# cloudflare/circl

Hardware: AMD Instinct MI355X
Metric: ML-KEM-768 encapsulations/sec (whole node), batch=2^20 (higher is better)
Workload: dtype i32; 1 GPU; ML-KEM-768 Encapsulate, distinct-key (one GPU-generated key per item), batch=1048576 per GPU, inputs resident in HBM (SURVEY 8d scope i; the PCIe-inclusive host-ABI rate, scope ii, is `value_host_abi`); key_pool=1048576, parallelism=batch split per device, no collectives, mode=encaps

## Files before the change

circl_amd/csrc/api_prims.hip:

```cpp
#include "host_common.h"
#include "prim_kernels.h"
#include "sampler_prims.h"

using namespace circl::host;

namespace {
PipeOpts prim_opts(size_t row_bytes) {
    PipeOpts o;
    o.chunk_items = host_chunk_items(std::max<size_t>(size_t(1) << 10, (size_t(32) << 20) / std::max<size_t>(row_bytes, 1)));
    return o;
}
const std::function<size_t(size_t)> no_ws = [](size_t) { return size_t(0); };
}

extern "C" {

int circl_hip_keccak_f1600(uint64_t *states, size_t n, int rounds, int device) {
    if (rounds != 24 && rounds != 12) return CIRCL_HIP_EPARAM;
    uint8_t *p = reinterpret_cast<uint8_t *>(states);
    return shard(n, device, [&](int dev, size_t lo, size_t cnt) {
        return run_pipeline(dev, cnt, {{p + lo * 200, 200}}, {}, {{p + lo * 200, 200}}, no_ws, prim_opts(200), [&](Chunk &c) {
            HIP_TRY(hipMemcpyAsync(c.out[0], c.in[0], c.cnt * 200, hipMemcpyDeviceToDevice, c.st));
            hipLaunchKernelGGL(circl::prim::keccak_f1600_kernel, dim3((unsigned)((c.cnt + 255) / 256)), dim3(256), 0, c.st,
                               reinterpret_cast<uint64_t *>(c.out[0]), c.cnt, 24 - rounds);
// ... 21 lines not shown
    auto timed = [&](auto kern, int iters, double insts_per_wave, double *out) -> int {
        float best = 1e30f;
        for (int rep = 0; rep < 4; rep++) {
            HIP_TRY(hipEventRecord(a, st));
            hipLaunchKernelGGL(kern, dim3((unsigned)(cus * waves_per_simd)), dim3(256), 0, st, sink, iters);
            HIP_TRY(hipEventRecord(b, st));
            HIP_TRY(hipEventSynchronize(b));
            float ms = 0;
            HIP_TRY(hipEventElapsedTime(&ms, a, b));
            if (rep > 0) best = std::min(best, ms);
        }
        if (out) *out = insts_per_wave * waves_per_simd / (best * 1e-3);
        return CIRCL_HIP_OK;
    };
    int rc = CIRCL_HIP_OK;
    if (hipEventCreate(&a) != hipSuccess || hipEventCreate(&b) != hipSuccess || hipStreamCreateWithFlags(&st, hipStreamNonBlocking) != hipSuccess) {
        (void)hipGetLastError();
        rc = CIRCL_HIP_EHIP;
    }
    constexpr int kKeccakIters = 512, kSimpleIters = 8192;
    if (rc == CIRCL_HIP_OK) rc = timed(circl::prim::keccak_rate_probe_kernel, kKeccakIters, 4320.0 * kKeccakIters, keccak_insts_per_s_per_simd);
    if (rc == CIRCL_HIP_OK) rc = timed(circl::prim::simple_rate_probe_kernel, kSimpleIters, (double)circl::prim::kSimpleProbePerIter * kSimpleIters, simple_insts_per_s_per_simd);
    cleanup();
    return rc;
}

int circl_hip_keccak_f1600_coop(uint64_t *states, size_t n, int device) {
    uint8_t *p = reinterpret_cast<uint8_t *>(states);
    return shard(n, device, [&](int dev, size_t lo, size_t cnt) {
        return run_pipeline(dev, cnt, {{p + lo * 200, 200}}, {}, {{p + lo * 200, 200}}, no_ws, prim_opts(200), [&](Chunk &c) {
            HIP_TRY(hipMemcpyAsync(c.out[0], c.in[0], c.cnt * 200, hipMemcpyDeviceToDevice, c.st));
            hipLaunchKernelGGL(circl::prim::keccak_f1600_coop_kernel, dim3((unsigned)c.cnt), dim3(64), 0, c.st, reinterpret_cast<uint64_t *>(c.out[0]));
            HIP_TRY(hipGetLastError());
            return CIRCL_HIP_OK;
        });
    });
}

int circl_hip_keccak_f1600_split(uint64_t *states, size_t n, int device) {
    uint8_t *p = reinterpret_cast<uint8_t *>(states);
    return shard(n, device, [&](int dev, size_t lo, size_t cnt) {
        return run_pipeline(dev, cnt, {{p + lo * 200, 200}}, {}, {{p + lo * 200, 200}}, no_ws, prim_opts(200), [&](Chunk &c) {
            HIP_TRY(hipMemcpyAsync(c.out[0], c.in[0], c.cnt * 200, hipMemcpyDeviceToDevice, c.st));
            hipLaunchKernelGGL(circl::prim::keccak_f1600_split_kernel, dim3((unsigned)((2 * c.cnt + 255) / 256)), dim3(256), 0, c.st,
                               reinterpret_cast<uint64_t *>(c.out[0]), c.cnt);
            HIP_TRY(hipGetLastError());
            return CIRCL_HIP_OK;
        });
    });
}

int circl_hip_kyber_ntt(int16_t *polys, size_t n, int inverse, int device) {
    uint8_t *p = reinterpret_cast<uint8_t *>(polys);
    return shard(n, device, [&](int dev, size_t lo, size_t cnt) {
        return run_pipeline(dev, cnt, {{p + lo * 512, 512}}, {}, {{p + lo * 512, 512}}, no_ws, prim_opts(512), [&](Chunk &c) {
            HIP_TRY(hipMemcpyAsync(c.out[0], c.in[0], c.cnt * 512, hipMemcpyDeviceToDevice, c.st));
            hipLaunchKernelGGL(circl::prim::kyber_ntt_kernel, dim3((unsigned)c.cnt), dim3(64), 0, c.st, reinterpret_cast<int16_t *>(c.out[0]), inverse);
            HIP_TRY(hipGetLastError());
            return CIRCL_HIP_OK;
        });
    });
}

int circl_hip_dilithium_ntt(uint32_t *polys, size_t n, int inverse, int device) {
    uint8_t *p = reinterpret_cast<uint8_t *>(polys);
    return shard(n, device, [&](int dev, size_t lo, size_t cnt) {
        return run_pipeline(dev, cnt, {{p + lo * 1024, 1024}}, {}, {{p + lo * 1024, 1024}}, no_ws, prim_opts(1024), [&](Chunk &c) {
            HIP_TRY(hipMemcpyAsync(c.out[0], c.in[0], c.cnt * 1024, hipMemcpyDeviceToDevice, c.st));
            hipLaunchKernelGGL(circl::prim::dilithium_ntt_kernel, dim3((unsigned)c.cnt), dim3(64), 0, c.st, reinterpret_cast<uint32_t *>(c.out[0]), inverse);
            HIP_TRY(hipGetLastError());
            return CIRCL_HIP_OK;
        });
    });
}

int circl_hip_kyber_mulhat(int16_t *out, const int16_t *a, const int16_t *b, size_t n, int device) {
    uint8_t *po = reinterpret_cast<uint8_t *>(out);
    const uint8_t *pa = reinterpret_cast<const uint8_t *>(a), *pb = reinterpret_cast<const uint8_t *>(b);
    return shard(n, device, [&](int dev, size_t lo, size_t cnt) {
        return run_pipeline(dev, cnt, {{pa + lo * 512, 512}, {pb + lo * 512, 512}}, {}, {{po + lo * 512, 512}}, no_ws, prim_opts(512), [&](Chunk &c) {
            hipLaunchKernelGGL(circl::prim::kyber_mulhat_kernel, dim3((unsigned)c.cnt), dim3(64), 0, c.st, reinterpret_cast<int16_t *>(c.out[0]),
                               reinterpret_cast<const int16_t *>(c.in[0]), reinterpret_cast<const int16_t *>(c.in[1]));
            HIP_TRY(hipGetLastError());
            return CIRCL_HIP_OK;
        });
    });
}

int circl_hip_shake(int rate, int ds, const uint8_t *in, size_t inlen, uint8_t *out, size_t outlen, size_t n, int device) {
    if ((rate != 168 && rate != 136 && rate != 72) || (ds != 0x1f && ds != 0x06) || outlen == 0) return CIRCL_HIP_EPARAM;
    const size_t il = inlen ? inlen : 1;
    std::vector<uint8_t> pad;
    const uint8_t *src = in;
    if (!inlen) { pad.assign(n, 0); src = pad.data(); }
    return shard(n, device, [&](int dev, size_t lo, size_t cnt) {
        return run_pipeline(dev, cnt, {{src + lo * il, il}}, {}, {{out + lo * outlen, outlen}}, no_ws, prim_opts(il + outlen), [&](Chunk &c) {
            hipLaunchKernelGGL(circl::prim::sponge_kernel, dim3((unsigned)((c.cnt + 255) / 256)), dim3(256), 0, c.st, rate / 8, (uint32_t)ds, 0,
                               (const uint8_t *)c.in[0], inlen, (const uint64_t *)nullptr, c.out[0], outlen, c.cnt);
            HIP_TRY(hipGetLastError());
            return CIRCL_HIP_OK;
        });
    });
}

int circl_hip_lane_op(int op, int arg, const uint32_t *a, const uint32_t *b, uint32_t *out0, uint32_t *out1, size_t n, int device) {
    if (op < 1 || op >= CIRCL_HIP_LANE_OP_COUNT || !a || !out0) return CIRCL_HIP_EPARAM;
    const uint8_t *pa = reinterpret_cast<const uint8_t *>(a), *pb = reinterpret_cast<const uint8_t *>(b);
    uint8_t *p0 = reinterpret_cast<uint8_t *>(out0), *p1 = reinterpret_cast<uint8_t *>(out1);
    return shard(n, device, [&](int dev, size_t lo, size_t cnt) {
        std::vector<HIn> ins = {{pa + lo * 4, 4}};
// ... 233 lines not shown
```

circl_amd/csrc/kyber_dev.h:

```cpp
#pragma once
#include "keccak_dev.h"

namespace circl {
namespace kyber {

constexpr int Q = 3329;
constexpr int N = 256;

CIRCL_HD int mul24(int a, int b) {
#if defined(__HIP_DEVICE_COMPILE__)
    return __mul24(a, b);
#else
    return a * b;
#endif
}
CIRCL_HD uint32_t umulhi32(uint32_t a, uint32_t b) {
#if defined(__HIP_DEVICE_COMPILE__)
    return __umulhi(a, b);
#else
    return (uint32_t)(((uint64_t)a * b) >> 32);
#endif
}

CIRCL_HD int barrett(int x) { return x - mul24(mul24(x, 20159) >> 26, Q); }
CIRCL_HD int csubq(int x) {
    x -= Q;
    return x + ((x >> 31) & Q);
}
CIRCL_HD int normalize(int x) { return csubq(barrett(x)); }

constexpr uint32_t qinv32() {
    uint32_t x = 1;
    for (int i = 0; i < 6; i++) x = x * (2u - (uint32_t)Q * x);
    return x;
}
constexpr uint32_t QINV32 = qinv32();
static_assert((uint32_t)(QINV32 * (uint32_t)Q) == 1u, "q * qinv == 1 mod 2^32");
constexpr uint32_t R32 = (uint32_t)((1ull << 32) % Q);
constexpr uint32_t MULC_LIMIT = (uint32_t)((1ull << 32) / Q);
constexpr uint32_t modq(int64_t x) { return (uint32_t)(((x % Q) + Q) % Q); }
constexpr uint32_t powq(uint32_t b, uint32_t e) {
    uint32_t r = 1;
    for (uint32_t i = 0; i < e; i++) r = r * b % Q;
    return r;
}
constexpr uint32_t invq(uint32_t x) { return powq(x % Q, Q - 2); }
constexpr uint32_t mulc_const(uint32_t w) { return modq(-(int64_t)((uint64_t)(w % Q) * R32 % Q)) * QINV32; }
CIRCL_HD uint32_t mulc(uint32_t b, uint32_t c) { return umulhi32(b * c, (uint32_t)Q); }
CIRCL_HD uint32_t reduce32(uint32_t t) { return umulhi32(t * QINV32, (uint32_t)Q); }
constexpr uint32_t NEG_R32 = modq(-(int64_t)R32);

struct ZetaTable {
    uint32_t w[128];
    uint32_t c[128];
// ... 21 lines not shown
CIRCL_HD uint32_t zeta_plain(int i) {
    constexpr ZetaTable t = make_zetas();
    return t.w[i];
}

struct LaneZetas {
    uint32_t f2, f3a, f3b, f4, f5a, f5b, f6, f6n;
    uint32_t i2, i3a, i3b, i4, i5a, i5b, i6;
};
CIRCL_HD LaneZetas load_lane_zetas(int lane) {
    LaneZetas z;
    const int h = lane >> 4, m = lane >> 2;
    z.f2 = zeta_c(4 + h);
    z.f3a = zeta_c(8 + 2 * h);
    z.f3b = zeta_c(9 + 2 * h);
    z.f4 = zeta_c(16 + m);
    z.f5a = zeta_c(32 + 2 * m);
    z.f5b = zeta_c(33 + 2 * m);
    z.f6 = zeta_c(64 + lane);
    z.f6n = zeta_cn(64 + lane);
    z.i2 = zeta_c(7 - h);
    z.i3a = zeta_c(15 - 2 * h);
    z.i3b = zeta_c(14 - 2 * h);
    z.i4 = zeta_c(31 - m);
    z.i5a = zeta_c(63 - 2 * m);
    z.i5b = zeta_c(62 - 2 * m);
    z.i6 = zeta_c(127 - lane);
    return z;
}

CIRCL_HD int idx_l1(int l, int r) { return l + 64 * r; }
CIRCL_HD int idx_l2(int l, int r) { return ((l >> 4) << 6) | (r << 4) | (l & 15); }
CIRCL_HD int idx_l3(int l, int r) { return ((l >> 2) << 4) | (r << 2) | (l & 3); }
CIRCL_HD int idx_l4(int l, int r) { return 4 * l + r; }

CIRCL_HD void ct(int &a, int &b, uint32_t c) {
    const int t = (int)mulc((uint32_t)b, c);
    b = a + Q - t;
    a = a + t;
}
template <int BOUND> CIRCL_HD void gs(int &a, int &b, uint32_t c) {
    const int t = b + BOUND - a;
    a = a + b;
    b = (int)mulc((uint32_t)t, c);
}

#if defined(__HIP_DEVICE_COMPILE__) || defined(__HIPCC__)

template <bool NW = false> __device__ __forceinline__ void wave_sync() {
    if constexpr (NW) wave_lds_order();
    else __syncthreads();
}

template <int FROM, int TO, class T, bool NW = false> __device__ __forceinline__ void relayout(int (&c)[4], void *xch_raw, int lane) {
    T *xch = reinterpret_cast<T *>(xch_raw);
    auto idx = [&](int which, int r) {
        return which == 1 ? idx_l1(lane, r) : which == 2 ? idx_l2(lane, r) : which == 3 ? idx_l3(lane, r) : idx_l4(lane, r);
    };
    wave_sync<NW>();
#pragma unroll
    for (int r = 0; r < 4; r++) xch[idx(FROM, r)] = (T)c[r];
    wave_sync<NW>();
#pragma unroll
    for (int r = 0; r < 4; r++) c[r] = (int)xch[idx(TO, r)];
}

template <bool NW = false> __device__ __forceinline__ void ntt(int (&c)[4], const LaneZetas &z, void *xch, int lane) {
    const uint32_t z1 = zeta_c(1), z2 = zeta_c(2), z3 = zeta_c(3);
    ct(c[0], c[2], z1); ct(c[1], c[3], z1);
    ct(c[0], c[1], z2); ct(c[2], c[3], z3);
    relayout<1, 2, uint16_t, NW>(c, xch, lane);
    ct(c[0], c[2], z.f2); ct(c[1], c[3], z.f2);
    ct(c[0], c[1], z.f3a); ct(c[2], c[3], z.f3b);
    relayout<2, 3, uint16_t, NW>(c, xch, lane);
    ct(c[0], c[2], z.f4); ct(c[1], c[3], z.f4);
    ct(c[0], c[1], z.f5a); ct(c[2], c[3], z.f5b);
    relayout<3, 4, uint16_t, NW>(c, xch, lane);
    ct(c[0], c[2], z.f6); ct(c[1], c[3], z.f6);
}

template <uint32_t SCALE, bool NW = false> __device__ __forceinline__ void invntt(int (&c)[4], const LaneZetas &z, void *xch, int lane) {
    static_assert(128u * Q < MULC_LIMIT, "lazy sums stay inside the mulc domain");
    gs<Q>(c[0], c[2], z.i6); gs<Q>(c[1], c[3], z.i6);
    relayout<4, 3, uint16_t, NW>(c, xch, lane);
    gs<2 * Q>(c[0], c[1], z.i5a); gs<2 * Q>(c[2], c[3], z.i5b);
    gs<4 * Q>(c[0], c[2], z.i4); gs<4 * Q>(c[1], c[3], z.i4);
    relayout<3, 2, uint16_t, NW>(c, xch, lane);
    gs<8 * Q>(c[0], c[1], z.i3a); gs<8 * Q>(c[2], c[3], z.i3b);
    gs<16 * Q>(c[0], c[2], z.i2); gs<16 * Q>(c[1], c[3], z.i2);
    relayout<2, 1, uint32_t, NW>(c, xch, lane);
    const uint32_t z1 = zeta_c(1), z2 = zeta_c(2), z3 = zeta_c(3);
    gs<32 * Q>(c[0], c[1], z3); gs<32 * Q>(c[2], c[3], z2);
    gs<64 * Q>(c[0], c[2], z1); gs<64 * Q>(c[1], c[3], z1);
    constexpr uint32_t fin = mulc_const((uint32_t)((uint64_t)(SCALE % Q) * invq(128) % Q));
#pragma unroll
    for (int r = 0; r < 4; r++) c[r] = (int)mulc((uint32_t)c[r], fin);
}
#endif

struct HatOperand {
    uint32_t p0, q0, p1, q1;
};
CIRCL_HD uint32_t pack16(int lo, int hi) { return ((uint32_t)lo & 0xffffu) | ((uint32_t)hi << 16); }
CIRCL_HD HatOperand hat_prepare(const int (&b)[4], uint32_t c_zeta, uint32_t c_neg_zeta) {
    HatOperand h;
    h.p0 = pack16(b[0], (int)mulc((uint32_t)b[1], c_zeta));
    h.q0 = pack16(b[1], b[0]);
    h.p1 = pack16(b[2], (int)mulc((uint32_t)b[3], c_neg_zeta));
    h.q1 = pack16(b[3], b[2]);
    return h;
}
CIRCL_HD int dot2(uint32_t a, uint32_t b, int c) {
#if defined(__HIP_DEVICE_COMPILE__)
    typedef short short2v __attribute__((ext_vector_type(2)));
    return __builtin_amdgcn_sdot2(__builtin_bit_cast(short2v, a), __builtin_bit_cast(short2v, b), c, false);
#else
    return (int)(int16_t)(a & 0xffff) * (int)(int16_t)(b & 0xffff) + (int)(int16_t)(a >> 16) * (int)(int16_t)(b >> 16) + c;
#endif
}
CIRCL_HD void mulhat_acc_packed(int (&acc)[4], uint32_t a01, uint32_t a23, const HatOperand &b) {
    acc[0] = dot2(a01, b.p0, acc[0]);
    acc[1] = dot2(a01, b.q0, acc[1]);
    acc[2] = dot2(a23, b.p1, acc[2]);
    acc[3] = dot2(a23, b.q1, acc[3]);
}
CIRCL_HD void mulhat_finish(int (&acc)[4]) {
#pragma unroll
    for (int r = 0; r < 4; r++) acc[r] = (int)reduce32((uint32_t)acc[r]);
}

CIRCL_HD int cbd2_from_nibble(unsigned t) {
    return (int)((t & 1) + ((t >> 1) & 1)) - (int)(((t >> 2) & 1) + ((t >> 3) & 1));
}
CIRCL_HD uint32_t cbd2_bias8_word(uint32_t w) {
    const uint32_t d = (w & 0x55555555u) + ((w >> 1) & 0x55555555u);
    return ((d & 0x33333333u) | 0x88888888u) - ((d >> 2) & 0x33333333u);
}
CIRCL_HD int cbd3_from_6bits(unsigned t) {
    return (int)((t & 1) + ((t >> 1) & 1) + ((t >> 2) & 1)) - (int)(((t >> 3) & 1) + ((t >> 4) & 1) + ((t >> 5) & 1));
}

template <int D> CIRCL_HD unsigned compress_coeff(int x) {
    static_assert(D == 4 || D == 5 || D == 10 || D == 11, "d");
// ... 16 lines not shown
```

circl_amd/csrc/mlkem_kernels.h:

```cpp
#pragma once
#include "kyber_dev.h"

#ifndef CIRCL_KEM_RING_PRIO
#define CIRCL_KEM_RING_PRIO 1
#endif
#ifndef CIRCL_KEM_WAVES_PER_EU
#define CIRCL_KEM_WAVES_PER_EU 4
#endif

namespace circl {
namespace mlkem {

using kyber::Q;

template <int K> struct Params;
template <> struct Params<2> { static constexpr int ETA1 = 3, DU = 10, DV = 4; };
template <> struct Params<3> { static constexpr int ETA1 = 2, DU = 10, DV = 4; };
template <> struct Params<4> { static constexpr int ETA1 = 2, DU = 11, DV = 5; };

template <int K> struct Geom {
    using P = Params<K>;
    static constexpr int EK = 384 * K + 32;
    static constexpr int DK = 768 * K + 96;
    static constexpr int CT = 32 * (P::DU * K + P::DV);
// ... 264 lines not shown
    const uint8_t *dkp = dk + idx * Gm::DK;
    KeccakState g;
    keccak_zero(g);
    xor_words<0, 4>(g, reinterpret_cast<const uint64_t *>(mprime_ws + idx * 32));
    xor_words<4, 4>(g, reinterpret_cast<const uint64_t *>(dkp + 768 * K + 32));
    g.lo[8] = kDsSha3;
    g.hi[8] = 0x80000000u;
    keccak_f1600(g);
    store_words<0, 4>(reinterpret_cast<uint64_t *>(kbar_ws + idx * 32), g);
    store_words<4, 4>(reinterpret_cast<uint64_t *>(r_ws + idx * 32), g);
    const uint64_t *zw = reinterpret_cast<const uint64_t *>(dkp + 768 * K + 64);
#pragma unroll
    for (int i = 0; i < 4; i++) reinterpret_cast<uint64_t *>(z_ws + idx * 32)[i] = zw[i];
    status[idx] = 0;
}


__device__ __forceinline__ void parse_shake128_block(const KeccakState &s, int16_t *poly, int &cnt) {
    detail::static_for<0, 112>([&](auto ic) {
        constexpr int c = decltype(ic)::v;
        constexpr int bit = 12 * c, w = bit / 32, sh = bit % 32;
        auto word = [&](int i) -> uint32_t { return (i & 1) ? s.hi[i >> 1] : s.lo[i >> 1]; };
        uint32_t v;
        if constexpr (sh <= 20) v = (word(w) >> sh) & 0xfffu;
        else v = alignbit(word(w + 1), word(w), sh) & 0xfffu;
        poly[cnt] = (int16_t)v;
        cnt = min(cnt + (v < (uint32_t)Q ? 1 : 0), 256);
    });
}

template <int K, bool TRANSPOSED>
__device__ __forceinline__ void sample_matrix(uint8_t *lds_a, const uint8_t *__restrict__ rho, size_t rho_stride, size_t item0,
                                              size_t n, int lane) {
    using Gm = Geom<K>;
    const bool on = lane < Gm::A_STREAMS;
    const int g = on ? lane / Gm::PAIRS : 0, p = on ? lane % Gm::PAIRS : 0;
    const int i = p / K, j = p % K;
    size_t item = item0 + g;
    if (item >= n) item = n - 1;
    KeccakState s;
    keccak_zero(s);
    xor_words<0, 4>(s, reinterpret_cast<const uint64_t *>(rho + item * rho_stride));
    s.lo[4] = (TRANSPOSED ? (uint32_t)i | ((uint32_t)j << 8) : (uint32_t)j | ((uint32_t)i << 8)) | (kDsShake << 16);
    s.hi[20] = 0x80000000u;
    int16_t *poly = reinterpret_cast<int16_t *>(lds_a + (on ? lane : 0) * Gm::A_STRIDE);
    int cnt = on ? 0 : 256;
#pragma unroll 1
    for (int blk = 0; blk < 3 || __any(cnt < 256); blk++) {
        keccak_f1600(s);
        if (on) parse_shake128_block(s, poly, cnt);
    }
}

template <bool TAIL, int SLOTS = 32>
__device__ __forceinline__ void parse_shake128_block_fifo(const KeccakState &s, int16_t *fifo, int16_t *row, int &cnt, int &flushed) {
    bool live = true;
    detail::static_for<0, 112>([&](auto ic) {
        constexpr int c = decltype(ic)::v;
        constexpr int bit = 12 * c, w = bit / 32, sh = bit % 32;
        auto word = [&](int i) -> uint32_t { return (i & 1) ? s.hi[i >> 1] : s.lo[i >> 1]; };
        if (!TAIL || live) {
            uint32_t v;
            if constexpr (sh <= 20) v = (word(w) >> sh) & 0xfffu;
            else v = alignbit(word(w + 1), word(w), sh) & 0xfffu;
            fifo[cnt & (SLOTS - 1)] = (int16_t)v;
            cnt += v < (uint32_t)Q ? 1 : 0;
            if constexpr (c % 8 == 7) {
                cnt = min(cnt, 256);
                if (cnt - flushed >= 8) {
                    const uint4 d = *reinterpret_cast<const uint4 *>(fifo + (flushed & (SLOTS - 1)));
                    *reinterpret_cast<uint4 *>(row + flushed) = d;
                    flushed += 8;
                }
                if constexpr (TAIL) live = __any(flushed < 256);
            }
        }
    });
}

template <int K, bool TRANSPOSED, int GA = Geom<K>::G, bool XY_ARG = false>
__device__ __forceinline__ void sample_matrix_scratch(uint8_t *lds_fifo, int16_t *rows, const uint8_t *__restrict__ rho,
                                                      size_t rho_stride, size_t item0, size_t n, int lane, const uint8_t *__restrict__ xy = nullptr) {
    using Gm = Geom<K>;
    const bool on = XY_ARG ? item0 + lane < n : lane < GA * Gm::PAIRS;
    const int g = XY_ARG ? lane : on ? lane / Gm::PAIRS : 0, p = on ? lane % Gm::PAIRS : 0;
    const int i = p / K, j = p % K;
    size_t item = item0 + g;
    if (item >= n) item = n - 1;
    KeccakState s;
    keccak_zero(s);
    xor_words<0, 4>(s, reinterpret_cast<const uint64_t *>(rho + item * rho_stride));
    if constexpr (XY_ARG) s.lo[4] = (uint32_t)xy[2 * item] | ((uint32_t)xy[2 * item + 1] << 8) | (kDsShake << 16);
    else s.lo[4] = (TRANSPOSED ? (uint32_t)i | ((uint32_t)j << 8) : (uint32_t)j | ((uint32_t)i << 8)) | (kDsShake << 16);
    s.hi[20] = 0x80000000u;
    int16_t *fifo = reinterpret_cast<int16_t *>(lds_fifo + lane * Gm::FIFO_STRIDE);
    int16_t *row = rows + lane * 256;
    int cnt = on ? 0 : 256, flushed = cnt;
#pragma unroll 1
    for (int blk = 0; blk < 3; blk++) {
        keccak_f1600(s);
        if (on) parse_shake128_block_fifo<false>(s, fifo, row, cnt, flushed);
    }
#pragma unroll 1
    while (__any(flushed < 256)) {
        keccak_f1600(s);
        parse_shake128_block_fifo<true>(s, fifo, row, cnt, flushed);
    }
}

template <bool ETA2> __device__ __forceinline__ void store_prf_words(uint32_t *out, const KeccakState &s) {
    detail::static_for<0, 16>([&](auto ic) {
        constexpr int w = decltype(ic)::v;
        out[2 * w] = ETA2 ? kyber::cbd2_bias8_word(s.lo[w]) : s.lo[w];
        out[2 * w + 1] = ETA2 ? kyber::cbd2_bias8_word(s.hi[w]) : s.hi[w];
    });
}

template <int K, bool TRANSPOSED, int NOISE, int ETA1_COUNT>
__device__ __forceinline__ void sample_matrix_and_prf(uint8_t *lds_fifo, uint8_t *lds_noise, uint8_t *lds_mini, int16_t *rows,
// ... 418 lines not shown
                __syncthreads();
                sample_matrix_scratch<K, true>(lds_a, rows, ek + 384 * K, ek_stride, item0, n, lane);
                __threadfence_block();
            } else {
                sample_matrix<K, true>(lds_a, ek + 384 * K, ek_stride, item0, n, lane);
            }
        }
        __syncthreads();
        if constexpr (Gm::HALVES == 1) {
            if (!(ABLATE & 2)) prf_streams<K, Gm::NOISE, K>(lds_noise, r_ws, 32, item0, n, lane);
            __syncthreads();
        }
    }

    int lane_ring = lane;
    asm volatile("" : "+v"(lane_ring));
    if constexpr (CIRCL_KEM_RING_PRIO != 0) __builtin_amdgcn_s_setprio(CIRCL_KEM_RING_PRIO);
    lap(1);
    const kyber::LaneZetas z = kyber::load_lane_zetas(lane_ring);
#pragma unroll 1
    for (int g = 0; g < ((ABLATE & 4) ? 0 : (int)gi); g++) {
        const size_t item = item0 + g;
        if (item >= n) break;
        if constexpr (Gm::HALVES > 1 && !SHARED) {
            if (g % Gm::GH == 0) {
                __syncthreads();
                if (!(ABLATE & 2)) prf_streams<K, Gm::NOISE, K, Gm::GH>(lds_noise, r_ws, 32, item0, n, lane, g);
                __syncthreads();
            }
        }
        const size_t kq = KM == KM_KEYED ? (key_idx ? (size_t)key_idx[item] : (ek_stride ? item : size_t(0))) : item;
        const uint8_t *ekp = ek + kq * ek_stride;
        const int16_t *krows = KM == KM_KEYED ? key_rows + kq * (size_t)(K * K * 256) : nullptr;
        const uint8_t *noise = lds_noise + (SHARED ? g : g % Gm::GH) * Gm::NOISE * Gm::NOISE_STRIDE;

        int th[K][4];
        bool bad = false;
#pragma unroll
        for (int j = 0; j < K; j++) {
            unpack12_l4(th[j], ekp + 384 * j, lane);
#pragma unroll
            for (int r = 0; r < 4; r++) {
                if (MODE == ENCAPS) bad |= th[j][r] >= Q;
                else th[j][r] = kyber::csubq(th[j][r]);
            }
        }
        const bool reject = MODE == ENCAPS ? __any(bad) : false;

        int rh[K][4];
#pragma unroll
        for (int j = 0; j < K; j++) {
#pragma unroll
            for (int r = 0; r < 4; r++) rh[j][r] = cbd_coeff<P::ETA1>(noise + j * Gm::NOISE_STRIDE, kyber::idx_l1(lane, r));
            kyber::ntt(rh[j], z, xch, lane);
        }
        kyber::HatOperand rop[K];
#pragma unroll
        for (int j = 0; j < K; j++) rop[j] = kyber::hat_prepare(rh[j], z.f6, z.f6n);

        uint8_t *ctp = ct + item * Gm::CT;
        bool differs = false;
#pragma unroll 1
        for (int i = 0; i < K; i++) {
            uint32_t *dst = reinterpret_cast<uint32_t *>(ctp + 32 * P::DU * i);
            RefWords<P::DU> ref;
            if (MODE == REENCRYPT) ref.load(dst, lane);
            int acc[4] = {0, 0, 0, 0};
#pragma unroll
            for (int j = 0; j < K; j++) {
                uint32_t a01, a23;
                if constexpr (KM == KM_KEYED) AFromCache{krows}.load(a01, a23, i * K + j, lane);
                else if constexpr (SCRATCH) AFromScratch{rows}.load(a01, a23, SHARED ? i * K + j : (g * K + i) * K + j, lane);
                else AFromLds{lds_a, Gm::A_STRIDE}.load(a01, a23, (g * K + i) * K + j, lane);
                kyber::mulhat_acc_packed(acc, a01, a23, rop[j]);
            }
            kyber::mulhat_finish(acc);
            kyber::invntt<kyber::NEG_R32>(acc, z, xch, lane);
            const uint8_t *e1 = noise + (K + i) * Gm::NOISE_STRIDE;
            unsigned cv[4];
#pragma unroll
            for (int r = 0; r < 4; r++)
                cv[r] = kyber::compress_coeff<P::DU>(acc[r] + cbd_coeff<2>(e1, kyber::idx_l1(lane, r)));
            uint32_t *stage = reinterpret_cast<uint32_t *>(xch);
            stage_bits_l1<P::DU>(stage, cv, lane);
            if (MODE == REENCRYPT) differs |= ref.differs(stage, lane);
            else store_staged<P::DU>(dst, stage, lane, reject);
        }
        {
            uint32_t *dst = reinterpret_cast<uint32_t *>(ctp + 32 * P::DU * K);
            RefWords<P::DV> ref;
            if (MODE == REENCRYPT) ref.load(dst, lane);
            int acc[4] = {0, 0, 0, 0};
#pragma unroll
            for (int j = 0; j < K; j++) kyber::mulhat_acc_packed(acc, kyber::pack16(th[j][0], th[j][1]), kyber::pack16(th[j][2], th[j][3]), rop[j]);
            kyber::mulhat_finish(acc);
            kyber::invntt<kyber::NEG_R32>(acc, z, xch, lane);
            const uint8_t *e2 = noise + 2 * K * Gm::NOISE_STRIDE;
            const uint8_t *mp = m + item * 32;
            unsigned cv[4];
#pragma unroll
            for (int r = 0; r < 4; r++) {
                const int nidx = kyber::idx_l1(lane, r);
                const int mbit = (mp[nidx >> 3] >> (nidx & 7)) & 1;
                cv[r] = kyber::compress_coeff<P::DV>(acc[r] + cbd_coeff<2>(e2, nidx) + (-mbit & ((Q + 1) / 2)));
            }
            uint32_t *stage = reinterpret_cast<uint32_t *>(xch);
            stage_bits_l1<P::DV>(stage, cv, lane);
            if (MODE == REENCRYPT) differs |= ref.differs(stage, lane);
            else store_staged<P::DV>(dst, stage, lane, reject);
        }
        if (MODE == ENCAPS) {
            if (lane == 0) status[item] = reject ? 1 : 0;
            if (reject && lane < 8) reinterpret_cast<uint32_t *>(ss + item * 32)[lane] = 0;
        } else if (MODE == REENCRYPT) {
            const bool mismatch = __any(differs);
            const bool dead = status[item] != 0;
            if (lane < 8) {
                const uint32_t kb = reinterpret_cast<const uint32_t *>(kbar_ws + item * 32)[lane];
                const uint32_t rj = reinterpret_cast<const uint32_t *>(ssrej_ws + item * 32)[lane];
                reinterpret_cast<uint32_t *>(ss + item * 32)[lane] = dead ? 0u : (mismatch ? rj : kb);
            }
        }
        if constexpr (CLK) clk[3]++;
    }
    lap(2);
  }
    if constexpr (CLK) {
        lap(0);
        if (lane == 0) {
            uint64_t *prof = reinterpret_cast<uint64_t *>(const_cast<int16_t *>(key_rows)) + (size_t)blockIdx.x * 4;
#pragma unroll
            for (int q = 0; q < 4; q++) prof[q] = clk[q];
        }
    }
}

template <int K>
__global__ void __launch_bounds__(64, CIRCL_KEM_WAVES_PER_EU) mlkem_expand_keys_kernel(const uint8_t *__restrict__ keys, size_t stride, size_t rho_off,
                                                                                      int16_t *__restrict__ key_rows, size_t nkeys) {
    using Gm = Geom<K>;
    extern __shared__ __attribute__((aligned(16))) uint8_t smem[];
    const size_t e0 = (size_t)blockIdx.x * Gm::G;
    sample_matrix_scratch<K, true>(smem, key_rows + e0 * (size_t)(K * K * 256), keys + rho_off, stride, e0, nkeys, threadIdx.x);
}

template <int K>
__device__ __forceinline__ void mlkem_hash_coop2(const uint8_t *__restrict__ ek, const uint8_t *__restrict__ m, uint8_t *__restrict__ ss,
                                                 uint8_t *__restrict__ r_ws, size_t item0, size_t n, uint64_t *ws, int lane) {
    using Gm = Geom<K>;
// ... 663 lines not shown
    extern __shared__ __attribute__((aligned(16))) uint8_t smem[];
    uint8_t *lds_a = smem;
    uint8_t *lds_noise = SCRATCH ? smem : smem + Gm::LDS_A;
    uint8_t *xch = lds_noise + Gm::LDS_NOISE;
    int16_t *rows = reinterpret_cast<int16_t *>(scratch + (size_t)blockIdx.x * Gm::SCRATCH_BYTES);
    const int lane = threadIdx.x;
    const kyber::LaneZetas z = kyber::load_lane_zetas(lane);
    const size_t ngroups = (n + Gm::G - 1) / Gm::G;

#pragma unroll 1
  for (size_t grp = next_group(work, lane, true, ngroups); grp < ngroups; grp = next_group(work, lane, false, ngroups)) {
    const size_t item0 = grp * Gm::G;
    if constexpr (CIRCL_KEM_RING_PRIO != 0) __builtin_amdgcn_s_setprio(0);
    if constexpr (SCRATCH && Gm::HALVES == 1) {
        __syncthreads();
        sample_matrix_and_prf<K, false, 2 * K, 2 * K>(lds_a, lds_noise, xch, rows, rs_ws, 64, rs_ws + 32, 64,
                                                      item0, n, lane);
        __threadfence_block();
        __syncthreads();
    } else {
        if constexpr (SCRATCH) {
            __syncthreads();
            sample_matrix_scratch<K, false>(lds_a, rows, rs_ws, 64, item0, n, lane);
            __threadfence_block();
        } else {
            sample_matrix<K, false>(lds_a, rs_ws, 64, item0, n, lane);
        }
        __syncthreads();
        if constexpr (Gm::HALVES == 1) {
            prf_streams<K, 2 * K, 2 * K>(lds_noise, rs_ws + 32, 64, item0, n, lane);
            __syncthreads();
        }
    }

    if constexpr (CIRCL_KEM_RING_PRIO != 0) __builtin_amdgcn_s_setprio(CIRCL_KEM_RING_PRIO);
#pragma unroll 1
    for (int g = 0; g < Gm::G; g++) {
        const size_t item = item0 + g;
        if (item >= n) break;
        if constexpr (Gm::HALVES > 1) {
            if (g % Gm::GH == 0) {
                __syncthreads();
                prf_streams<K, 2 * K, 2 * K, Gm::GH>(lds_noise, rs_ws + 32, 64, item0, n, lane, g);
                __syncthreads();
            }
        }
        const uint8_t *noise = lds_noise + (g % Gm::GH) * (2 * K) * Gm::NOISE_STRIDE;
        uint8_t *ekp = ek + item * Gm::EK, *dkp = dk + item * Gm::DK;
        int sh[K][4];
#pragma unroll
        for (int j = 0; j < K; j++) {
#pragma unroll
            for (int r = 0; r < 4; r++) sh[j][r] = cbd_coeff<P::ETA1>(noise + j * Gm::NOISE_STRIDE, kyber::idx_l1(lane, r));
            kyber::ntt(sh[j], z, xch, lane);
#pragma unroll
            for (int r = 0; r < 4; r++) sh[j][r] = kyber::normalize(sh[j][r]);
            pack12_l4(dkp + 384 * j, sh[j], lane);
        }
        kyber::HatOperand sop[K];
#pragma unroll
        for (int j = 0; j < K; j++) sop[j] = kyber::hat_prepare(sh[j], z.f6, z.f6n);
#pragma unroll 1
        for (int i = 0; i < K; i++) {
            int eh[4], acc[4] = {0, 0, 0, 0};
#pragma unroll
            for (int r = 0; r < 4; r++) eh[r] = cbd_coeff<P::ETA1>(noise + (K + i) * Gm::NOISE_STRIDE, kyber::idx_l1(lane, r));
            kyber::ntt(eh, z, xch, lane);
#pragma unroll
            for (int j = 0; j < K; j++) {
                uint32_t a01, a23;
                if constexpr (SCRATCH) AFromScratch{rows}.load(a01, a23, (g * K + i) * K + j, lane);
                else AFromLds{lds_a, Gm::A_STRIDE}.load(a01, a23, (g * K + i) * K + j, lane);
                kyber::mulhat_acc_packed(acc, a01, a23, sop[j]);
            }
            kyber::mulhat_finish(acc);
            int t[4];
#pragma unroll
            for (int r = 0; r < 4; r++)
                t[r] = kyber::normalize((int)kyber::mulc((uint32_t)acc[r], kyber::mulc_const(kyber::NEG_R32)) + eh[r]);
            pack12_l4(ekp + 384 * i, t, lane);
            pack12_l4(dkp + 384 * K + 384 * i, t, lane);
        }
        if (lane < 8) {
            const uint32_t w = reinterpret_cast<const uint32_t *>(rs_ws + item * 64)[lane];
            reinterpret_cast<uint32_t *>(ekp + 384 * K)[lane] = w;
            reinterpret_cast<uint32_t *>(dkp + 768 * K)[lane] = w;
        }
    }
  }
}

template <int K>
__global__ void __launch_bounds__(256) mlkem_keygen_finish_kernel(const uint8_t *__restrict__ seed64, const uint8_t *__restrict__ ek,
                                                                  uint8_t *__restrict__ dk, size_t n) {
    using Gm = Geom<K>;
    size_t idx = (size_t)blockIdx.x * 256 + threadIdx.x;
    const bool live = idx < n;
    if (!live) idx = n - 1;
    KeccakState h;
    sha3_256_words<Gm::EK / 8>(h, reinterpret_cast<const uint64_t *>(ek + idx * Gm::EK));
    if (live) {
        uint64_t *tail = reinterpret_cast<uint64_t *>(dk + idx * Gm::DK + 768 * K + 32);
        store_words<0, 4>(tail, h);
        const uint64_t *zsrc = reinterpret_cast<const uint64_t *>(seed64 + idx * 64 + 32);
#pragma unroll
        for (int i = 0; i < 4; i++) tail[4 + i] = zsrc[i];
    }
}

template <int K>
__global__ void __launch_bounds__(64) mlkem_keygen_finish_small_kernel(const uint8_t *__restrict__ seed64, const uint8_t *__restrict__ ek,
                                                                       uint8_t *__restrict__ dk, size_t n, int form) {
    using Gm = Geom<K>;
    __shared__ uint64_t ws[100];
    const int lane = threadIdx.x;
    if (form == 1) {
        const int half = lane >> 5, j = lane & 31;
        size_t idx = 2 * (size_t)blockIdx.x + half;
        const bool live = idx < n;
        if (!live) idx = n - 1;
// ... 154 lines not shown
```

circl_amd/csrc/prim_kernels.h:

```cpp
#pragma once
#include "kyber_dev.h"
#include "dilithium_dev.h"
#include "lane_ops.h"

namespace circl {
namespace prim {

__global__ void __launch_bounds__(256) keccak_f1600_kernel(uint64_t *states, size_t n, int first_round) {
    const size_t i = (size_t)blockIdx.x * 256 + threadIdx.x;
    if (i >= n) return;
    uint64_t *p = states + i * 25;
    KeccakState s;
#pragma unroll
    for (int w = 0; w < 25; w++) { s.lo[w] = (uint32_t)p[w]; s.hi[w] = (uint32_t)(p[w] >> 32); }
    keccak_f1600(s, first_round);
#pragma unroll
    for (int w = 0; w < 25; w++) p[w] = ((uint64_t)s.hi[w] << 32) | s.lo[w];
}

__global__ void __launch_bounds__(256) keccak_rate_probe_kernel(uint32_t *sink, int iters) {
    KeccakState s;
#pragma unroll
    for (int w = 0; w < 25; w++) { s.lo[w] = threadIdx.x * 2654435761u + w; s.hi[w] = blockIdx.x * 40503u ^ (w << 7); }
#pragma unroll 1
    for (int i = 0; i < iters; i++) keccak_f1600(s, 0);
    uint32_t x = 0;
#pragma unroll
    for (int w = 0; w < 25; w++) x ^= s.lo[w] ^ s.hi[w];
    if (x == 0x12345678u) sink[0] = x;
}
constexpr int kSimpleProbePerIter = 256;
__global__ void __launch_bounds__(256) simple_rate_probe_kernel(uint32_t *sink, int iters) {
    uint32_t a0 = threadIdx.x, a1 = a0 + 1, a2 = a0 + 2, a3 = a0 + 3, a4 = a0 + 4, a5 = a0 + 5, a6 = a0 + 6, a7 = a0 + 7;
    const uint32_t b = threadIdx.x * 2654435761u + blockIdx.x;
#pragma unroll 1
    for (int i = 0; i < iters; i++) {
#pragma unroll
        for (int r = 0; r < kSimpleProbePerIter / 8; r++)
            asm volatile("v_add_u32 %0, %0, %8\n v_xor_b32 %1, %1, %8\n v_add_u32 %2, %2, %8\n v_xor_b32 %3, %3, %8\n"
                         "v_add_u32 %4, %4, %8\n v_xor_b32 %5, %5, %8\n v_add_u32 %6, %6, %8\n v_xor_b32 %7, %7, %8"
                         : "+v"(a0), "+v"(a1), "+v"(a2), "+v"(a3), "+v"(a4), "+v"(a5), "+v"(a6), "+v"(a7)
                         : "v"(b));
    }
    if ((a0 ^ a1 ^ a2 ^ a3 ^ a4 ^ a5 ^ a6 ^ a7) == 0x12345678u) sink[0] = a0;
}

__global__ void __launch_bounds__(64) keccak_f1600_coop_kernel(uint64_t *states) {
    __shared__ uint64_t ws[55];
    const int lane = threadIdx.x;
    uint64_t *p = states + (size_t)blockIdx.x * 25;
    if (lane < 25) ws[lane] = p[lane];
    keccak_f1600_coop(ws, lane);
    if (lane < 25) p[lane] = ws[lane];
}

__global__ void __launch_bounds__(256) keccak_f1600_split_kernel(uint64_t *states, size_t n) {
    const size_t lane = (size_t)blockIdx.x * 256 + threadIdx.x;
    size_t item = lane >> 1;
    const int p = (int)(lane & 1);
    const bool live = item < n;
    if (!live) item = n - 1;
    uint32_t *w = reinterpret_cast<uint32_t *>(states + item * 25);
    SplitState s;
#pragma unroll
    for (int k = 0; k < 25; k++) s.w[k] = w[2 * k + p];
    keccak_f1600_split(s, p != 0);
    if (live) {
#pragma unroll
        for (int k = 0; k < 25; k++) w[2 * k + p] = s.w[k];
    }
}

__global__ void __launch_bounds__(64) kyber_ntt_kernel(int16_t *polys, int inverse) {
    __shared__ __attribute__((aligned(16))) uint32_t xch[256];
    const int lane = threadIdx.x;
    int16_t *p = polys + (size_t)blockIdx.x * 256;
    const kyber::LaneZetas z = kyber::load_lane_zetas(lane);
    int c[4];
    if (!inverse) {
#pragma unroll
        for (int r = 0; r < 4; r++) c[r] = kyber::normalize(p[kyber::idx_l1(lane, r)]);
        kyber::ntt(c, z, xch, lane);
#pragma unroll
        for (int r = 0; r < 4; r++) p[kyber::idx_l4(lane, r)] = (int16_t)kyber::normalize(c[r]);
    } else {
#pragma unroll
        for (int r = 0; r < 4; r++) c[r] = kyber::normalize(p[kyber::idx_l4(lane, r)]);
        kyber::invntt<65536u>(c, z, xch, lane);
#pragma unroll
        for (int r = 0; r < 4; r++) p[kyber::idx_l1(lane, r)] = (int16_t)c[r];
    }
}

__global__ void __launch_bounds__(64) kyber_mulhat_kernel(int16_t *out, const int16_t *a, const int16_t *b) {
    const int lane = threadIdx.x;
    const size_t off = (size_t)blockIdx.x * 256 + 4 * lane;
    int x[4], y[4], acc[4] = {0, 0, 0, 0};
#pragma unroll
    for (int r = 0; r < 4; r++) { x[r] = kyber::normalize(a[off + r]); y[r] = kyber::normalize(b[off + r]); }
    kyber::mulhat_acc_packed(acc, kyber::pack16(x[0], x[1]), kyber::pack16(x[2], x[3]), kyber::hat_prepare(y, kyber::zeta_c(64 + lane), kyber::zeta_cn(64 + lane)));
    kyber::mulhat_finish(acc);
    constexpr uint32_t fix = kyber::mulc_const(kyber::modq((int64_t)kyber::NEG_R32 * kyber::invq(65536u % kyber::Q)));
#pragma unroll
    for (int r = 0; r < 4; r++) out[off + r] = (int16_t)kyber::mulc((uint32_t)acc[r], fix);
}

__global__ void __launch_bounds__(64) dilithium_ntt_kernel(uint32_t *polys, int inverse) {
    __shared__ __attribute__((aligned(16))) uint32_t xch[dilithium::kXchWords];
    const int lane = threadIdx.x;
    uint32_t *p = polys + (size_t)blockIdx.x * 256;
    const dilithium::LaneZetas z = dilithium::load_lane_zetas(lane);
    uint32_t c[4];
    if (!inverse) {
#pragma unroll
        for (int r = 0; r < 4; r++) c[r] = dilithium::normalize(p[kyber::idx_l1(lane, r)]);
        dilithium::ntt(c, z, xch, lane);
#pragma unroll
        for (int r = 0; r < 4; r++) p[kyber::idx_l4(lane, r)] = dilithium::normalize(c[r]);
    } else {
#pragma unroll
        for (int r = 0; r < 4; r++) c[r] = dilithium::normalize(p[kyber::idx_l4(lane, r)]);
        dilithium::invntt(c, z, xch, lane);
#pragma unroll
        for (int r = 0; r < 4; r++) p[kyber::idx_l1(lane, r)] = dilithium::normalize(dilithium::mont32(c[r], dilithium::R32SQ));
    }
}

__global__ void __launch_bounds__(256) sponge_kernel(int rate_words, uint32_t ds, int first_round, const uint8_t *in, size_t inlen_eq,
                                                     const uint64_t *in_off, uint8_t *out, size_t outlen, size_t n,
                                                     const uint64_t *in_len = nullptr, uint64_t suffix = 0) {
    const size_t i = (size_t)blockIdx.x * 256 + threadIdx.x;
    if (i >= n) return;
    const uint8_t *p = in_off ? in + in_off[i] : in + i * inlen_eq;
    const size_t body = in_len ? (size_t)(in_len[i] & 0x00ffffffffffffffull) : in_off ? (size_t)(in_off[i + 1] - in_off[i]) : inlen_eq;
    const size_t inlen = body + (in_len ? (size_t)(in_len[i] >> 56) : 0);
    uint8_t *o = out + i * outlen;
    const size_t rate = (size_t)rate_words * 8;
    KeccakState s;
    keccak_zero(s);
    size_t pos = 0;
    bool padded = false;
// ... 66 lines not shown
```

Measured before the change: 140.1 million encaps/s.

## Replace LDS relayouts in Kyber NTT with cross-lane permute/DPP swaps

Adds cross-lane exchange variants (permlane32/16 swap and DPP row/quad ops) that transpose coefficient layouts between NTT stages within registers, replacing the LDS store/barrier/load round trips. The default is now the lane-only variant for ML-KEM encaps and keygen, and the prim NTT kernel is templated with an env selector. It also adds an inline-asm compare-and-add-with-carry for rejection-sampling accept counting. This removes LDS traffic and barriers per relayout, at the cost of relying on gfx950-specific permlane builtins and on the lane-mapping correctness of the transposes.

```diff
diff --git a/circl_amd/csrc/api_prims.hip b/circl_amd/csrc/api_prims.hip
--- a/circl_amd/csrc/api_prims.hip
+++ b/circl_amd/csrc/api_prims.hip
@@ -97,10 +97,15 @@
 
 int circl_hip_kyber_ntt(int16_t *polys, size_t n, int inverse, int device) {
     uint8_t *p = reinterpret_cast<uint8_t *>(polys);
+    const int xch = env_int("CIRCL_HIP_NTT_XCH", CIRCL_KEM_RING_XCH, 0, 3);
+    auto *kern = xch == circl::kyber::XCH_LDS      ? circl::prim::kyber_ntt_kernel<circl::kyber::XCH_LDS>
+                 : xch == circl::kyber::XCH_LDS_NW ? circl::prim::kyber_ntt_kernel<circl::kyber::XCH_LDS_NW>
+                 : xch == circl::kyber::XCH_LANES  ? circl::prim::kyber_ntt_kernel<circl::kyber::XCH_LANES>
+                                                   : circl::prim::kyber_ntt_kernel<circl::kyber::XCH_LANES_TOP>;
     return shard(n, device, [&](int dev, size_t lo, size_t cnt) {
         return run_pipeline(dev, cnt, {{p + lo * 512, 512}}, {}, {{p + lo * 512, 512}}, no_ws, prim_opts(512), [&](Chunk &c) {
             HIP_TRY(hipMemcpyAsync(c.out[0], c.in[0], c.cnt * 512, hipMemcpyDeviceToDevice, c.st));
-            hipLaunchKernelGGL(circl::prim::kyber_ntt_kernel, dim3((unsigned)c.cnt), dim3(64), 0, c.st, reinterpret_cast<int16_t *>(c.out[0]), inverse);
+            hipLaunchKernelGGL(kern, dim3((unsigned)c.cnt), dim3(64), 0, c.st, reinterpret_cast<int16_t *>(c.out[0]), inverse);
             HIP_TRY(hipGetLastError());
             return CIRCL_HIP_OK;
         });
diff --git a/circl_amd/csrc/kyber_dev.h b/circl_amd/csrc/kyber_dev.h
--- a/circl_amd/csrc/kyber_dev.h
+++ b/circl_amd/csrc/kyber_dev.h
@@ -1,5 +1,9 @@
 #pragma once
 #include "keccak_dev.h"
+
+#ifndef CIRCL_KEM_RING_XCH
+#define CIRCL_KEM_RING_XCH 2
+#endif
 
 namespace circl {
 namespace kyber {
@@ -127,43 +131,88 @@
     else __syncthreads();
 }
 
-template <int FROM, int TO, class T, bool NW = false> __device__ __forceinline__ void relayout(int (&c)[4], void *xch_raw, int lane) {
-    T *xch = reinterpret_cast<T *>(xch_raw);
-    auto idx = [&](int which, int r) {
-        return which == 1 ? idx_l1(lane, r) : which == 2 ? idx_l2(lane, r) : which == 3 ? idx_l3(lane, r) : idx_l4(lane, r);
-    };
-    wave_sync<NW>();
-#pragma unroll
-    for (int r = 0; r < 4; r++) xch[idx(FROM, r)] = (T)c[r];
-    wave_sync<NW>();
-#pragma unroll
-    for (int r = 0; r < 4; r++) c[r] = (int)xch[idx(TO, r)];
-}
-
-template <bool NW = false> __device__ __forceinline__ void ntt(int (&c)[4], const LaneZetas &z, void *xch, int lane) {
+enum Exchange { XCH_LDS = 0, XCH_LDS_NW = 1, XCH_LANES = 2, XCH_LANES_TOP = 3 };
+
+template <int B> __device__ __forceinline__ void lane_swap(int &a, int &b, int lane) {
+    static_assert(B >= 0 && B <= 5, "lane bit");
+    constexpr int ROW_SHL = 0x100, ROW_SHR = 0x110, ROW_ROR = 0x120;
+    if constexpr (B == 5) {
+        const auto v = __builtin_amdgcn_permlane32_swap((unsigned)a, (unsigned)b, false, false);
+        a = (int)v[0];
+        b = (int)v[1];
+    } else if constexpr (B == 4) {
+        const auto v = __builtin_amdgcn_permlane16_swap((unsigned)a, (unsigned)b, false, false);
+        a = (int)v[0];
+        b = (int)v[1];
+    } else if constexpr (B == 3) {
+        const int t = a;
+        a = __builtin_amdgcn_update_dpp(a, b, ROW_ROR + 8, 0xf, 0xc, false);
+        b = __builtin_amdgcn_update_dpp(b, t, ROW_ROR + 8, 0xf, 0x3, false);
+    } else if constexpr (B == 2) {
+        const int t = a;
+        a = __builtin_amdgcn_update_dpp(a, b, ROW_SHR + 4, 0xf, 0xa, false);
+        b = __builtin_amdgcn_update_dpp(b, t, ROW_SHL + 4, 0xf, 0x5, false);
+    } else {
+        constexpr int QUAD = B == 1 ? 0x4e : 0xb1;
+        const bool up = (lane >> B) & 1;
+        const int send = up ? a : b;
+        const int recv = __builtin_amdgcn_update_dpp(0, send, QUAD, 0xf, 0xf, true);
+        a = up ? recv : a;
+        b = up ? b : recv;
+    }
+}
+template <int HI> __device__ __forceinline__ void lane_transpose(int (&c)[4], int lane) {
+    lane_swap<HI>(c[0], c[2], lane);
+    lane_swap<HI>(c[1], c[3], lane);
+    lane_swap<HI - 1>(c[0], c[1], lane);
+    lane_swap<HI - 1>(c[2], c[3], lane);
+}
+
+template <int FROM, int TO, class T, int XCH = XCH_LDS> __device__ __forceinline__ void relayout(int (&c)[4], void *xch_raw, int lane) {
+    constexpr int LOW = FROM < TO ? FROM : TO;
+    static_assert(XCH >= XCH_LDS && XCH <= XCH_LANES_TOP, "exchange form");
+    if constexpr (XCH == XCH_LANES || (XCH == XCH_LANES_TOP && LOW == 1)) {
+        static_assert(FROM - TO == 1 || TO - FROM == 1, "cross-lane exchanges are between neighbouring layouts");
+        lane_transpose<7 - 2 * LOW>(c, lane);
+    } else {
+        constexpr bool NW = XCH == XCH_LDS_NW;
+        T *xch = reinterpret_cast<T *>(xch_raw);
+        auto idx = [&](int which, int r) {
+            return which == 1 ? idx_l1(lane, r) : which == 2 ? idx_l2(lane, r) : which == 3 ? idx_l3(lane, r) : idx_l4(lane, r);
+        };
+        wave_sync<NW>();
+#pragma unroll
+        for (int r = 0; r < 4; r++) xch[idx(FROM, r)] = (T)c[r];
+        wave_sync<NW>();
+#pragma unroll
+        for (int r = 0; r < 4; r++) c[r] = (int)xch[idx(TO, r)];
+    }
+}
+
+template <int XCH = XCH_LDS> __device__ __forceinline__ void ntt(int (&c)[4], const LaneZetas &z, void *xch, int lane) {
     const uint32_t z1 = zeta_c(1), z2 = zeta_c(2), z3 = zeta_c(3);
     ct(c[0], c[2], z1); ct(c[1], c[3], z1);
     ct(c[0], c[1], z2); ct(c[2], c[3], z3);
-    relayout<1, 2, uint16_t, NW>(c, xch, lane);
+    relayout<1, 2, uint16_t, XCH>(c, xch, lane);
     ct(c[0], c[2], z.f2); ct(c[1], c[3], z.f2);
     ct(c[0], c[1], z.f3a); ct(c[2], c[3], z.f3b);
-    relayout<2, 3, uint16_t, NW>(c, xch, lane);
+    relayout<2, 3, uint16_t, XCH>(c, xch, lane);
     ct(c[0], c[2], z.f4); ct(c[1], c[3], z.f4);
     ct(c[0], c[1], z.f5a); ct(c[2], c[3], z.f5b);
-    relayout<3, 4, uint16_t, NW>(c, xch, lane);
+    relayout<3, 4, uint16_t, XCH>(c, xch, lane);
     ct(c[0], c[2], z.f6); ct(c[1], c[3], z.f6);
 }
 
-template <uint32_t SCALE, bool NW = false> __device__ __forceinline__ void invntt(int (&c)[4], const LaneZetas &z, void *xch, int lane) {
+template <uint32_t SCALE, int XCH = XCH_LDS> __device__ __forceinline__ void invntt(int (&c)[4], const LaneZetas &z, void *xch, int lane) {
     static_assert(128u * Q < MULC_LIMIT, "lazy sums stay inside the mulc domain");
     gs<Q>(c[0], c[2], z.i6); gs<Q>(c[1], c[3], z.i6);
-    relayout<4, 3, uint16_t, NW>(c, xch, lane);
+    relayout<4, 3, uint16_t, XCH>(c, xch, lane);
     gs<2 * Q>(c[0], c[1], z.i5a); gs<2 * Q>(c[2], c[3], z.i5b);
     gs<4 * Q>(c[0], c[2], z.i4); gs<4 * Q>(c[1], c[3], z.i4);
-    relayout<3, 2, uint16_t, NW>(c, xch, lane);
+    relayout<3, 2, uint16_t, XCH>(c, xch, lane);
     gs<8 * Q>(c[0], c[1], z.i3a); gs<8 * Q>(c[2], c[3], z.i3b);
     gs<16 * Q>(c[0], c[2], z.i2); gs<16 * Q>(c[1], c[3], z.i2);
-    relayout<2, 1, uint32_t, NW>(c, xch, lane);
+    relayout<2, 1, uint32_t, XCH>(c, xch, lane);
     const uint32_t z1 = zeta_c(1), z2 = zeta_c(2), z3 = zeta_c(3);
     gs<32 * Q>(c[0], c[1], z3); gs<32 * Q>(c[2], c[3], z2);
     gs<64 * Q>(c[0], c[2], z1); gs<64 * Q>(c[1], c[3], z1);
diff --git a/circl_amd/csrc/mlkem_kernels.h b/circl_amd/csrc/mlkem_kernels.h
--- a/circl_amd/csrc/mlkem_kernels.h
+++ b/circl_amd/csrc/mlkem_kernels.h
@@ -340,6 +340,17 @@
     }
 }
 
+#ifndef CIRCL_KEM_ACCEPT_ASM
+#define CIRCL_KEM_ACCEPT_ASM 1
+#endif
+__device__ __forceinline__ void count_accept(int &cnt, uint32_t v) {
+#if defined(__HIP_DEVICE_COMPILE__) && CIRCL_KEM_ACCEPT_ASM
+    asm("v_cmp_gt_u32_e32 vcc, %2, %1\n\tv_addc_co_u32_e32 %0, vcc, 0, %0, vcc" : "+v"(cnt) : "v"(v), "s"((uint32_t)Q) : "vcc");
+#else
+    cnt += v < (uint32_t)Q ? 1 : 0;
+#endif
+}
+
 template <bool TAIL, int SLOTS = 32>
 __device__ __forceinline__ void parse_shake128_block_fifo(const KeccakState &s, int16_t *fifo, int16_t *row, int &cnt, int &flushed) {
     bool live = true;
@@ -352,7 +363,7 @@
             if constexpr (sh <= 20) v = (word(w) >> sh) & 0xfffu;
             else v = alignbit(word(w + 1), word(w), sh) & 0xfffu;
             fifo[cnt & (SLOTS - 1)] = (int16_t)v;
-            cnt += v < (uint32_t)Q ? 1 : 0;
+            count_accept(cnt, v);
             if constexpr (c % 8 == 7) {
                 cnt = min(cnt, 256);
                 if (cnt - flushed >= 8) {
@@ -877,7 +888,7 @@
         for (int j = 0; j < K; j++) {
 #pragma unroll
             for (int r = 0; r < 4; r++) rh[j][r] = cbd_coeff<P::ETA1>(noise + j * Gm::NOISE_STRIDE, kyber::idx_l1(lane, r));
-            kyber::ntt(rh[j], z, xch, lane);
+            kyber::ntt<CIRCL_KEM_RING_XCH>(rh[j], z, xch, lane);
         }
         kyber::HatOperand rop[K];
 #pragma unroll
@@ -900,7 +911,7 @@
                 kyber::mulhat_acc_packed(acc, a01, a23, rop[j]);
             }
             kyber::mulhat_finish(acc);
-            kyber::invntt<kyber::NEG_R32>(acc, z, xch, lane);
+            kyber::invntt<kyber::NEG_R32, CIRCL_KEM_RING_XCH>(acc, z, xch, lane);
             const uint8_t *e1 = noise + (K + i) * Gm::NOISE_STRIDE;
             unsigned cv[4];
 #pragma unroll
@@ -919,7 +930,7 @@
 #pragma unroll
             for (int j = 0; j < K; j++) kyber::mulhat_acc_packed(acc, kyber::pack16(th[j][0], th[j][1]), kyber::pack16(th[j][2], th[j][3]), rop[j]);
             kyber::mulhat_finish(acc);
-            kyber::invntt<kyber::NEG_R32>(acc, z, xch, lane);
+            kyber::invntt<kyber::NEG_R32, CIRCL_KEM_RING_XCH>(acc, z, xch, lane);
             const uint8_t *e2 = noise + 2 * K * Gm::NOISE_STRIDE;
             const uint8_t *mp = m + item * 32;
             unsigned cv[4];
@@ -1689,7 +1700,7 @@
         for (int j = 0; j < K; j++) {
 #pragma unroll
             for (int r = 0; r < 4; r++) sh[j][r] = cbd_coeff<P::ETA1>(noise + j * Gm::NOISE_STRIDE, kyber::idx_l1(lane, r));
-            kyber::ntt(sh[j], z, xch, lane);
+            kyber::ntt<CIRCL_KEM_RING_XCH>(sh[j], z, xch, lane);
 #pragma unroll
             for (int r = 0; r < 4; r++) sh[j][r] = kyber::normalize(sh[j][r]);
             pack12_l4(dkp + 384 * j, sh[j], lane);
@@ -1702,7 +1713,7 @@
             int eh[4], acc[4] = {0, 0, 0, 0};
 #pragma unroll
             for (int r = 0; r < 4; r++) eh[r] = cbd_coeff<P::ETA1>(noise + (K + i) * Gm::NOISE_STRIDE, kyber::idx_l1(lane, r));
-            kyber::ntt(eh, z, xch, lane);
+            kyber::ntt<CIRCL_KEM_RING_XCH>(eh, z, xch, lane);
 #pragma unroll
             for (int j = 0; j < K; j++) {
                 uint32_t a01, a23;
diff --git a/circl_amd/csrc/prim_kernels.h b/circl_amd/csrc/prim_kernels.h
--- a/circl_amd/csrc/prim_kernels.h
+++ b/circl_amd/csrc/prim_kernels.h
@@ -71,7 +71,7 @@
     }
 }
 
-__global__ void __launch_bounds__(64) kyber_ntt_kernel(int16_t *polys, int inverse) {
+template <int XCH> __global__ void __launch_bounds__(64) kyber_ntt_kernel(int16_t *polys, int inverse) {
     __shared__ __attribute__((aligned(16))) uint32_t xch[256];
     const int lane = threadIdx.x;
     int16_t *p = polys + (size_t)blockIdx.x * 256;
@@ -80,13 +80,13 @@
     if (!inverse) {
 #pragma unroll
         for (int r = 0; r < 4; r++) c[r] = kyber::normalize(p[kyber::idx_l1(lane, r)]);
-        kyber::ntt(c, z, xch, lane);
+        kyber::ntt<XCH>(c, z, xch, lane);
 #pragma unroll
         for (int r = 0; r < 4; r++) p[kyber::idx_l4(lane, r)] = (int16_t)kyber::normalize(c[r]);
     } else {
 #pragma unroll
         for (int r = 0; r < 4; r++) c[r] = kyber::normalize(p[kyber::idx_l4(lane, r)]);
-        kyber::invntt<65536u>(c, z, xch, lane);
+        kyber::invntt<65536u, XCH>(c, z, xch, lane);
 #pragma unroll
         for (int r = 0; r < 4; r++) p[kyber::idx_l1(lane, r)] = (int16_t)c[r];
     }
```

Measured after the change: 142.1 million encaps/s (median of 6 runs). 1.5% higher.
